# JeffOwOSun/ntm-tracker

Measured on AMD Instinct MI355X. Metric: frames/sec (whole node) VGG16+NTM(128x20) seq_len=20, higher is better.
Workload: dtype f32

## Files before the change

### include/ntmtrack.h

```cpp
#ifndef NTMTRACK_H_
#define NTMTRACK_H_

#include <stddef.h>
#include <stdint.h>

#ifdef __cplusplus
extern "C" {
#endif

#define NTK_OK               0
#define NTK_ERR_BAD_SHAPE   -1
#define NTK_ERR_BAD_PTR     -2
#define NTK_ERR_UNSUPPORTED -3
#define NTK_ERR_HIP         -4

int ntk_version(void);
const char* ntk_last_error(void);


int ntk_vgg_packed_k(int cin);
int ntk_vgg_pack_weights(const float* w_hwio, float* w_packed, int cin, int cout, void* stream);

int ntk_vgg_conv3x3_relu_f32(const float* in, const float* w_packed, const float* bias,
                             float* out, int frames, int H, int W, int cin, int cout,
// ... 29 lines not shown
int ntk_vgg_pack_weights_wino43(const float* w_hwio, float* u_packed, int cin, int cout, void* stream);
int ntk_vgg_conv3x3_relu_wino43_f32(const float* in, const float* u_packed, const float* bias, float* out,
                                    int frames, int H, int W, int cin, int cout, int fuse_pool, void* stream);
int ntk_vgg_conv3x3_relu_wino43_window_f32(const float* in, const float* u_packed, const float* bias, float* out,
                                           int frames, int H, int W, int cin, int cout, int fuse_pool,
                                           int y0, int x0, int y1, int x1, void* stream);
int ntk_vgg_conv3x3_relu_wino43_form_f32(const float* in, const float* u_packed, const float* bias, float* out,
                                         int frames, int H, int W, int cin, int cout, int fuse_pool,
                                         int y0, int x0, int y1, int x1, int waves, void* stream);
int ntk_vgg_conv3x3_relu_wino43_layout_f32(const float* in, const float* u_packed, const float* bias, float* out,
                                           int frames, int H, int W, int cin, int cout, int fuse_pool,
                                           int in_blocked, int out_blocked, void* stream);

int ntk_maxpool2x2(const float* in, float* out, int frames, int H, int W, int C, void* stream);


int ntk_gemm_nt_f32(const float* A, int lda, const float* B, int ldb, const float* bias,
                    float* C, int ldc, int M, int N, int K, void* stream);

size_t ntk_gemm_tn_workspace_bytes(int M, int N, int splits);
int ntk_gemm_tn_f32(const float* A, int lda, const float* B, int ldb, float* C, int ldc,
                    int M, int N, int K, int splits, int accumulate, float* workspace,
                    void* stream);

int ntk_transpose_pad(const float* in, int ldi, float* out, int ldo, int rows, int cols, void* stream);


int ntk_ntm_padded_dims(int N, int Md, int R, int Wh, int hid, int shift_range, int O,
                        int* P, int* PP, int* K, int* ldz, int* ldh);

#define NTK_NTM_FWD_WS           1
#define NTK_NTM_FWD_FIX512       2
#define NTK_NTM_FWD_GENERIC768   3
#define NTK_NTM_FWD_GENERIC1024  4
#define NTK_NTM_FWD_FIX640_DEV   5
#define NTK_NTM_BWD_WS           1
#define NTK_NTM_BWD_FIX          2
#define NTK_NTM_BWD_GENERIC768   3
#define NTK_NTM_BWD_GENERIC1024  4
#define NTK_NTM_PLAN_FWD 1
#define NTK_NTM_PLAN_BWD 2

int ntk_ntm_seq_plan(int B, int N, int Md, int R, int Wh, int hid, int shift_range, int O, int write_first,
                     int ldkT, int ldhT, int* fwd_kernel, int* fwd_threads, int* bwd_kernel, int* bwd_threads);

int ntk_ntm_seq_fwd(int B, int S, int N, int Md, int R, int Wh, int hid, int shift_range, int O,
// ... 128 lines not shown
                             float* st_wc, float* st_wv, float* st_w, float* st_M, float* st_read,
                             float* st_xtop, float* st_buf0, float* st_bufk, float* st_lgates, float* st_lc,
                             void* stream);
int ntk_ntm_seq_bwd_deep_sim(int B, int S, int N, int Md, int R, int Wh, int hid, int shift_range, int O, int L,
                             int write_first, int similarity,
                             const float* Wb, const float* WaT, int ldhT,
                             const float* M0, const float* w0, const float* cs0,
                             const float* st_gates, const float* st_c, const float* st_u,
                             const float* st_wc, const float* st_wv, const float* st_w, const float* st_M,
                             const float* st_lgates, const float* st_lc,
                             const float* dlogits,
                             const float* dM_fin, const float* dw_fin, const float* dread_fin, const float* dcs_fin,
                             float* dgates, float* dpre, float* du, float* dM0, float* dw0, float* dread0, float* dcs0,
                             void* stream);

int ntk_lstm_step_fwd(const float* pre, const float* c_prev, float forget_bias, float* c, float* h, float* act,
                      int B, int hid, void* stream);
int ntk_lstm_step_bwd(const float* act, const float* c_prev, const float* c, const float* dh, const float* dc,
                      float* dpre, float* dc_prev, int B, int hid, void* stream);

int ntk_ntm_init_state(const float* v, float* out, int n, int B, int act, void* stream);
int ntk_ntm_init_state_bwd(const float* v, const float* dout, float* dv, int n, int B, int act,
                           int accumulate, void* stream);

int ntk_dnc_padded_dims(int N, int W, int R, int Wn, int hid, int O,
                        int* I, int* IP, int* K, int* ldz, int* ldh, int* Ky, int* ldy, int* OP);
int ntk_dnc_seq_fwd(int B, int S, int N, int W, int R, int Wn, int hid, int O, float clip_value,
                    const float* xproj, const float* Wr, const float* Wi, const float* Wy,
                    float* mem, float* link, float* usage, float* rw, float* ww, float* prec,
                    float* reads, float* hc, float* out,
                    float* rec_z, float* rec_gates, float* rec_c, float* rec_hc, float* rec_yin,
                    float* rec_ifc, float* rec_u, float* rec_ww, float* rec_rw, float* rec_cw,
                    float* rec_cr, float* rec_al, float* rec_p, float* rec_fwd, float* rec_bwd,
                    float* rec_M, float* rec_L, float* rec_ypre, void* stream);

int ntk_dnc_cluster_plan(int B, int N, int W, int R, int Wn, int hid, int O, int k_request, int* k, size_t* workspace_bytes);
int ntk_dnc_cluster_status(const void* workspace, int B, int k, void* stream);
int ntk_dnc_cluster_placement(const void* workspace, int B, int k, int* same_xcd_clusters, void* stream);
int ntk_dnc_cluster_guard(const void* workspace, size_t workspace_bytes, int mp_form, int B, int k, float* loss, float* grad,
                          size_t n, void* stream);
int ntk_dnc_cluster_inject_abort(void* workspace, size_t workspace_bytes, int mp_form, int B, int k, void* stream);
int ntk_dnc_cluster_fwd(int B, int S, int N, int W, int R, int Wn, int hid, int O, float clip_value, int k,
                        const float* xproj, const float* Wr, const float* Wi, const float* Wy,
                        float* mem, float* link, float* usage, float* rw, float* ww, float* prec,
                        float* reads, float* hc, float* out,
                        float* rec_z, float* rec_gates, float* rec_c, float* rec_hc, float* rec_yin,
// ... 166 lines not shown
```

### ntm-tracker_amd/_lib.py

```python
import ctypes
import os

import torch

_HERE = os.path.dirname(os.path.abspath(__file__))
LIB_PATH = os.environ.get("NTK_LIB_PATH") or os.path.join(_HERE, "libntmtrack_hip.so")

_lib = None


class NtkError(RuntimeError):
    pass


def _sig(lib):
    c_int, c_void_p, c_size_t = ctypes.c_int, ctypes.c_void_p, ctypes.c_size_t
    P = c_void_p
    sigs = {
        "ntk_version": (c_int, []),
        "ntk_last_error": (ctypes.c_char_p, []),
        "ntk_vgg_packed_k": (c_int, [c_int]),
        "ntk_vgg_pack_weights": (c_int, [P, P, c_int, c_int, P]),
        "ntk_vgg_conv3x3_relu_f32": (c_int, [P, P, P, P, c_int, c_int, c_int, c_int, c_int, c_int, P]),
        "ntk_vgg_pack_weights_bf16": (c_int, [P, P, c_int, c_int, P]),
        "ntk_vgg_conv3x3_relu_bf16": (c_int, [P, P, P, P] + [c_int] * 7 + [P]),
        "ntk_vgg_conv3x3_relu_f32_to_bf16": (c_int, [P, P, P, P] + [c_int] * 5 + [P]),
        "ntk_vgg_bf16p_packed_elems": (c_size_t, [c_int, c_int]),
        "ntk_vgg_bf16p_supported": (c_int, [c_int] * 5),
        "ntk_vgg_pack_weights_bf16p": (c_int, [P, P] + [c_int] * 4 + [P]),
        "ntk_vgg_conv3x3_relu_bf16p": (c_int, [P, P, P, P] + [c_int] * 7 + [P]),
        "ntk_vgg_split3_packed_elems": (c_size_t, [c_int, c_int]),
        "ntk_vgg_split3_supported": (c_int, [c_int] * 5),
        "ntk_vgg_pack_weights_split3": (c_int, [P, P] + [c_int] * 4 + [P]),
        "ntk_vgg_conv3x3_relu_split3": (c_int, [P, P, P, P] + [c_int] * 8 + [P]),
        "ntk_gemm_nt_f32": (c_int, [P, c_int, P, c_int, P, P, c_int, c_int, c_int, c_int, P]),
        "ntk_gemm_tn_workspace_bytes": (c_size_t, [c_int, c_int, c_int]),
        "ntk_gemm_tn_f32": (c_int, [P, c_int, P, c_int, P, c_int, c_int, c_int, c_int, c_int, c_int, P, P]),
        "ntk_ntm_padded_dims": (c_int, [c_int] * 7 + [ctypes.POINTER(c_int)] * 5),
        "ntk_ntm_seq_fwd": (c_int, [c_int] * 10 + [P] * 23 + [P]),
        "ntk_transpose_pad": (c_int, [P, c_int, P, c_int, c_int, c_int, P]),
        "ntk_ntm_seq_bwd": (c_int, [c_int] * 10 + [P, c_int, P, c_int] + [P] * 21 + [P]),
        "ntk_ntm_seq_deep_supported": (c_int, [c_int] * 9),
        "ntk_ntm_seq_plan": (c_int, [c_int] * 11 + [ctypes.POINTER(c_int)] * 4),
        "ntk_ntm_seq_deep_plan": (c_int, [c_int] * 10 + [ctypes.POINTER(c_int)] * 4),
        "ntk_ntm_seq_deep_packed_floats": (c_int, [c_int] * 5 + [ctypes.POINTER(c_size_t)] * 3),
        "ntk_ntm_seq_deep_pack": (c_int, [c_int] * 5 + [P] * 6 + [P]),
        "ntk_ntm_seq_fwd_deep": (c_int, [c_int] * 12 + [P] * 29 + [P]),
        "ntk_ntm_seq_bwd_deep": (c_int, [c_int] * 11 + [P, P, c_int] + [P] * 24 + [P]),
        "ntk_dnc_padded_dims": (c_int, [c_int] * 6 + [ctypes.POINTER(c_int)] * 8),
        "ntk_dnc_seq_fwd": (c_int, [c_int] * 8 + [ctypes.c_float] + [P] * 13 + [P] * 18 + [P]),
        "ntk_dnc_cluster_plan": (c_int, [c_int] * 8 + [ctypes.POINTER(c_int), ctypes.POINTER(c_size_t)]),
        "ntk_dnc_cluster_status": (c_int, [P, c_int, c_int, P]),
        "ntk_dnc_cluster_placement": (c_int, [P, c_int, c_int, P, P]),
        "ntk_dnc_cluster_guard": (c_int, [P, c_size_t, c_int, c_int, c_int, P, P, c_size_t, P]),
        "ntk_dnc_cluster_inject_abort": (c_int, [P, c_size_t, c_int, c_int, c_int, P]),
        "ntk_dnc_cluster_fwd": (c_int, [c_int] * 8 + [ctypes.c_float, c_int] + [P] * 13 + [P] * 18 + [P, P]),
        "ntk_dnc_cluster_bwd_plan": (c_int, [c_int] * 8 + [ctypes.POINTER(c_int), ctypes.POINTER(c_size_t)]),
        "ntk_dnc_cluster_bwd": (c_int, [c_int] * 8 + [ctypes.c_float, c_int] + [P, c_int, P, P] + [P] * 7 + [P] * 15 + [P] * 6 + [P, c_int, P, P]),
        "ntk_cu_count": (c_int, []),
        "ntk_dnc_mp_plan": (c_int, [c_int] * 8 + [ctypes.POINTER(c_int), ctypes.POINTER(c_size_t)]),
# ... 45 lines not shown
        "ntk_vgg_conv3x3_relu_wino43_form_f32": (c_int, [P] * 4 + [c_int] * 11 + [P]),
        "ntk_vgg_conv3x3_relu_wino43_layout_f32": (c_int, [P] * 4 + [c_int] * 8 + [P]),
        "ntk_maxpool2x2": (c_int, [P, P] + [c_int] * 4 + [P]),
        "ntk_offset_loss_fwd": (c_int, [P] * 4 + [c_int] * 4 + [P]),
        "ntk_offset_loss_bwd": (c_int, [P] * 3 + [c_int] * 4 + [P]),
        "ntk_dnc_seq_bwd": (c_int, [c_int] * 8 + [ctypes.c_float] + [P, c_int, P, c_int, P] + [P] * 7 + [P] * 15 + [P] * 6 + [P, c_int, P]),
        "ntk_gather_serialize": (c_int, [P, P, P] + [c_int] * 9 + [P]),
        "ntk_gather_serialize_online": (c_int, [P, P, P] + [c_int] * 9 + [P]),
        "ntk_crop_and_resize": (c_int, [P, c_int, c_int, c_int, P] + [ctypes.c_float] * 4 + [P, c_int, c_int, ctypes.c_float, P]),
        "ntk_crop_and_resize_batch": (c_int, [P] + [c_int] * 5 + [P, P, P, P] + [c_int] * 3 + [ctypes.c_float, P]),
        "ntk_track_boxes_update": (c_int, [P, c_int, c_int, ctypes.c_double, ctypes.c_double] + [P] * 6 + [P]),
        "ntk_track_overlap_scores": (c_int, [P, P, P, P, c_int, c_int, c_int, P, c_int, P, c_int, P, P, P]),
        "ntk_select_rows": (c_int, [P, P, P, P, c_int, c_int, P]),
        "ntk_dnc_state_keep": (c_int, [P, c_int, c_int, c_int, P, P, P, P]),
        "ntk_resize_bilinear": (c_int, [P, c_int, c_int, c_int, P, c_int, c_int, P]),
        "ntk_offset_loss": (c_int, [P, P, P, P, P, c_int, c_int, c_int, c_int, P]),
        "ntk_log_loss": (c_int, [P, P, P, P, c_int, P]),
        "ntk_serialize_sequential": (c_int, [P, P, P] + [c_int] * 5 + [P]),
        "ntk_heatmap_ce_loss": (c_int, [P] * 5 + [c_int] * 3 + [P]),
        "ntk_serialize_two_step": (c_int, [P, P, P] + [c_int] * 5 + [P]),
        "ntk_two_step_ce_loss": (c_int, [P] * 5 + [c_int] * 3 + [P]),
        "ntk_ntm_init_state": (c_int, [P, P, c_int, c_int, c_int, P]),
        "ntk_ntm_init_state_bwd": (c_int, [P, P, P, c_int, c_int, c_int, c_int, P]),
        "ntk_global_norm_workspace_bytes": (c_size_t, [c_size_t]),
        "ntk_global_norm": (c_int, [P, c_size_t, P, P, P]),
        "ntk_rmsprop_clip_step": (c_int, [P, P, P, P, c_size_t] + [ctypes.c_float] * 5 + [P, P]),
        "ntk_rmsprop_clip_step_checked": (c_int, [P, P, P, P, c_size_t] + [ctypes.c_float] * 5 + [P, P, P, P]),
    }
    for name, (res, args) in sigs.items():
        fn = getattr(lib, name)
        fn.restype = res
        fn.argtypes = args
    return sigs


def lib():
    global _lib
    if _lib is None:
        if not os.path.exists(LIB_PATH):
            raise NtkError(
                "libntmtrack_hip.so is not built (%s). Run `python -c 'import __graft_entry__ as g; g.build()'` "
                "or `make -C ntm-tracker_amd/csrc`. There is no CPU fallback." % LIB_PATH)
        l = ctypes.CDLL(LIB_PATH)
        l._ntk_sigs = _sig(l)
        _lib = l
    return _lib
# ... 25 lines not shown
```

### ntm-tracker_amd/csrc/head_opt.hip

```cpp
#include "common.h"

namespace {

__global__ void gather_serialize_kernel(const float* __restrict__ fmap, const float* __restrict__ gts0,
                                        float* __restrict__ X, int T, int Hf, int Wf, int C, int ldx,
                                        int g0, int gstep, int gn, int delim_first) {
    const int NF = gn * gn;
    const int row = blockIdx.x;
    const int pos = row % (NF + 1);
    const int i = delim_first ? (pos == 0 ? NF : pos - 1) : pos;
    const int ft = row / (NF + 1);
    const int t = ft % T, b = ft / T;
    float* xr = X + (size_t)row * ldx;
    const int C4 = C >> 2;
    if (i < NF) {
        const int y = g0 + (i / gn) * gstep, x = g0 + (i % gn) * gstep;
        const f32x4* src = reinterpret_cast<const f32x4*>(fmap + (((size_t)ft * Hf + y) * Wf + x) * C);
        f32x4* dst = reinterpret_cast<f32x4*>(xr);
        for (int c = threadIdx.x; c < C4; c += blockDim.x) dst[c] = src[c];
    } else {
        f32x4 z = {0.f, 0.f, 0.f, 0.f};
        f32x4* dst = reinterpret_cast<f32x4*>(xr);
        for (int c = threadIdx.x; c < C4; c += blockDim.x) dst[c] = z;
    }
// ... 180 lines not shown
}

__global__ __launch_bounds__(1024) void log_loss_kernel(const float* __restrict__ logits, const float* __restrict__ labels,
                                                         float* __restrict__ loss, float* __restrict__ dlogits, int n) {
    __shared__ float red[16];
    const float eps = 1e-7f, inv = 1.0f / (float)n;
    float acc = 0.f;
    for (int i = threadIdx.x; i < n; i += blockDim.x) {
        const float p = 1.0f / (1.0f + expf(-logits[i]));
        const float y = labels[i];
        acc += -(y * logf(p + eps) + (1.0f - y) * logf(1.0f - p + eps));
        if (dlogits) dlogits[i] = inv * (-(y / (p + eps)) + (1.0f - y) / (1.0f - p + eps)) * p * (1.0f - p);
    }
    acc = wave_sum(acc);
    if ((threadIdx.x & 63) == 0) red[threadIdx.x >> 6] = acc;
    __syncthreads();
    if (threadIdx.x == 0) {
        float s = 0.f;
        for (int w = 0; w < (int)(blockDim.x >> 6); ++w) s += red[w];
        *loss = s * inv;
    }
}

__global__ void init_state_kernel(const float* __restrict__ v, float* __restrict__ out, int n, int B, int act) {
    const int i = blockIdx.x * blockDim.x + threadIdx.x;
    if (i >= n) return;
    const float x = v[i];
    const float y = act ? 1.0f / (1.0f + expf(-x)) : tanhf(x);
    for (int b = 0; b < B; ++b) out[(size_t)b * n + i] = y;
}

__global__ void init_state_bwd_kernel(const float* __restrict__ v, const float* __restrict__ dout,
                                      float* __restrict__ dv, int n, int B, int act, int accumulate) {
    const int i = blockIdx.x * blockDim.x + threadIdx.x;
    if (i >= n) return;
    float s = 0.f;
    for (int b = 0; b < B; ++b) s += dout[(size_t)b * n + i];
    const float x = v[i];
    float dy;
    if (act) { const float y = 1.0f / (1.0f + expf(-x)); dy = y * (1.0f - y); }
    else { const float y = tanhf(x); dy = 1.0f - y * y; }
    const float g = s * dy;
    dv[i] = accumulate ? dv[i] + g : g;
}

constexpr int SUMSQ_BLOCK = 256;
constexpr int SUMSQ_PER_BLOCK = 4096;

__global__ void sumsq_partial_kernel(const float* __restrict__ g, float* __restrict__ partial, size_t n) {
    __shared__ float red[SUMSQ_BLOCK / 64];
    const size_t base = (size_t)blockIdx.x * SUMSQ_PER_BLOCK;
    float acc = 0.f;
    for (int i = threadIdx.x; i < SUMSQ_PER_BLOCK; i += SUMSQ_BLOCK) {
        const size_t idx = base + i;
        if (idx < n) { const float v = g[idx]; acc += v * v; }
    }
    acc = wave_sum(acc);
    if ((threadIdx.x & 63) == 0) red[threadIdx.x >> 6] = acc;
    __syncthreads();
    if (threadIdx.x == 0) {
        float s = 0.f;
        for (int w = 0; w < SUMSQ_BLOCK / 64; ++w) s += red[w];
        partial[blockIdx.x] = s;
    }
}

// ... 442 lines not shown
    const unsigned nb = (unsigned)((total + 255) / 256 < 4096 ? (total + 255) / 256 : 4096);
    serialize_two_step_kernel<<<nb, 256, 0, (hipStream_t)stream>>>(feat, target, X, B, T, D, F, ldx);
    NTK_CHECK_LAUNCH("ntk_serialize_two_step");
    return NTK_OK;
}

extern "C" int ntk_two_step_ce_loss(const float* logits, const float* gt, float* probs, float* loss, float* dlogits,
                                    int B, int T, int F, void* stream) {
    NTK_REQUIRE(logits && gt && (loss || dlogits || probs), NTK_ERR_BAD_PTR, "ntk_two_step_ce_loss: null pointer");
    NTK_REQUIRE(B > 0 && T >= 1 && F > 0, NTK_ERR_BAD_SHAPE, "ntk_two_step_ce_loss: B=%d T=%d F=%d", B, T, F);
    two_step_ce_loss_kernel<<<1, 1024, 0, (hipStream_t)stream>>>(logits, gt, probs, loss, dlogits, B, T, F);
    NTK_CHECK_LAUNCH("ntk_two_step_ce_loss");
    return NTK_OK;
}

extern "C" int ntk_ntm_init_state(const float* v, float* out, int n, int B, int act, void* stream) {
    NTK_REQUIRE(v && out, NTK_ERR_BAD_PTR, "ntk_ntm_init_state: null pointer");
    NTK_REQUIRE(n > 0 && B > 0 && (act == 0 || act == 1), NTK_ERR_BAD_SHAPE, "ntk_ntm_init_state: n=%d B=%d act=%d", n, B, act);
    init_state_kernel<<<(n + 255) / 256, 256, 0, (hipStream_t)stream>>>(v, out, n, B, act);
    NTK_CHECK_LAUNCH("ntk_ntm_init_state");
    return NTK_OK;
}

extern "C" int ntk_ntm_init_state_bwd(const float* v, const float* dout, float* dv, int n, int B, int act,
                                      int accumulate, void* stream) {
    NTK_REQUIRE(v && dout && dv, NTK_ERR_BAD_PTR, "ntk_ntm_init_state_bwd: null pointer");
    NTK_REQUIRE(n > 0 && B > 0 && (act == 0 || act == 1), NTK_ERR_BAD_SHAPE, "ntk_ntm_init_state_bwd: n=%d B=%d act=%d", n, B, act);
    init_state_bwd_kernel<<<(n + 255) / 256, 256, 0, (hipStream_t)stream>>>(v, dout, dv, n, B, act, accumulate);
    NTK_CHECK_LAUNCH("ntk_ntm_init_state_bwd");
    return NTK_OK;
}

extern "C" size_t ntk_global_norm_workspace_bytes(size_t n) {
    return ((n + SUMSQ_PER_BLOCK - 1) / SUMSQ_PER_BLOCK) * sizeof(float);
}

extern "C" int ntk_global_norm(const float* grads, size_t n, float* workspace, float* gnorm, void* stream) {
    NTK_REQUIRE(grads && workspace && gnorm, NTK_ERR_BAD_PTR, "ntk_global_norm: null pointer");
    NTK_REQUIRE(n > 0, NTK_ERR_BAD_SHAPE, "ntk_global_norm: n=0");
    const int nb = (int)((n + SUMSQ_PER_BLOCK - 1) / SUMSQ_PER_BLOCK);
    sumsq_partial_kernel<<<nb, SUMSQ_BLOCK, 0, (hipStream_t)stream>>>(grads, workspace, n);
    NTK_CHECK_LAUNCH("ntk_global_norm(partial)");
    sumsq_final_kernel<<<1, 1024, 0, (hipStream_t)stream>>>(workspace, nb, gnorm);
    NTK_CHECK_LAUNCH("ntk_global_norm(final)");
    return NTK_OK;
}
// ... 25 lines not shown
```

### ntm-tracker_amd/dnc.py

```python
import collections
import ctypes

import torch

from . import _lib
from .ntm import gemm_nt, gemm_tn

_P = _lib.ptr

DNCState = collections.namedtuple("DNCState", ("access_output", "access_state", "controller_state"))
AccessState = collections.namedtuple("AccessState", ("memory", "read_weights", "write_weights", "linkage", "usage"))
TemporalLinkageState = collections.namedtuple("TemporalLinkageState", ("link", "precedence_weights"))
LSTMState = collections.namedtuple("LSTMState", ("hidden", "cell"))

INTERFACE = ("write_vectors", "erase_vectors", "free_gate", "allocation_gate", "write_gate", "read_mode",
             "write_keys", "write_strengths", "read_keys", "read_strengths")


class FlatParams(object):

    def __init__(self, shapes, device):
        n = 0
        self.shapes = list(shapes)
        self.offsets = {}
        for name, shp in shapes:
            sz = 1
            for s_ in shp:
                sz *= s_
            n = (n + 3) // 4 * 4
# ... 431 lines not shown
            return _P(keep[-1])
        recs = (_P(rec["gates"]), _P(rec["c"]), _P(rec["ifc"]), _P(rec["u"]), _P(rec["ww"]), _P(rec["rw"]), _P(rec["cw"]),
                _P(rec["cr"]), _P(rec["al"]), _P(rec["p"]), _P(rec["fwd"]), _P(rec["bwd"]), _P(rec["M"]), _P(rec["L"]),
                _P(rec["ypre"]), _P(dout), _P(gM), _P(gL), _P(dgates), _P(dxi), _P(dypre),
                _P(gcarry) if gcarry is not None else None, 1 if carry_in else 0)
        state0 = (c(acc.memory), c(acc.linkage.link), c(acc.usage), c(acc.read_weights), c(acc.write_weights),
                  c(acc.linkage.precedence_weights), _P(hc0))
        plan = self._cluster_bwd_plan(B)
        self.last_cluster_bwd_k = plan[1] if plan else 1
        self.last_cluster_bwd_form = plan[0] if plan else None
        if plan:
            fn = _lib.lib().ntk_dnc_cluster_bwd if plan[0] == "lds" else _lib.lib().ntk_dnc_mp_bwd
            _lib.check(fn(B, S, self.N, self.W, self.R, self.Wn, hid, self.O, self.clip_value, plan[1],
                          _P(WrT), ldkT, _P(self.Wi), _P(self.Wy), *state0, *recs, _P(plan[2]), _lib.stream()),
                       "ntk_dnc_cluster_bwd" if plan[0] == "lds" else "ntk_dnc_mp_bwd")
        else:
            _lib.check(_lib.lib().ntk_dnc_seq_bwd(
                B, S, self.N, self.W, self.R, self.Wn, hid, self.O, self.clip_value,
                _P(WrT), ldkT, _P(WiT), ldhT, _P(self.Wy), *state0, *recs, _lib.stream()), "ntk_dnc_seq_bwd")
        return dgates, dxi, dypre

    def _weight_grads(self, X2, rec, dgates, dxi, dypre, BS, accumulate):
        P, hid = self.params, self.hid
        gemm_tn(dgates.view(BS, 4 * hid), X2, P.view("WxT", grad=True), accumulate=accumulate)
        gemm_tn(rec["z"].view(BS, self.ldz), dgates.view(BS, 4 * hid), P.view("Wr", grad=True), accumulate=accumulate)
        gemm_tn(rec["hc"].view(BS, self.ldh), dxi.view(BS, self.IP), P.view("Wi", grad=True), accumulate=accumulate)
        gemm_tn(rec["yin"].view(BS, self.ldy), dypre.view(BS, self.OP), P.view("Wy", grad=True), accumulate=accumulate)

    def backward_sequence(self, X, dout, unpack=True):
        if not 1 <= self.Wn <= 4:
            raise _lib.NtkError("DNC BPTT on the HIP path implements 1..4 write heads (got %d)" % self.Wn)
        rec, st0 = self.last_record, self.last_initial
        if not rec and not self.last_segments:
            raise _lib.NtkError("backward_sequence needs a recorded forward pass (record=True)")
        B, S, _ = X.shape
        dev, L, stream = self.device, _lib.lib(), _lib.stream()
        hid = self.hid
        ldkT, ldhT = (self.K + 3) // 4 * 4, (hid + 3) // 4 * 4
        WrT = torch.empty((4 * hid, ldkT), device=dev)
        WiT = torch.empty((self.IP, ldhT), device=dev)
        _lib.check(L.ntk_transpose_pad(_P(self.Wr), 4 * hid, _P(WrT), ldkT, self.K, 4 * hid, stream), "ntk_transpose_pad")
        _lib.check(L.ntk_transpose_pad(_P(self.Wi), self.IP, _P(WiT), ldhT, hid, self.IP, stream), "ntk_transpose_pad")
        gM = torch.zeros((B, self.N, self.W), device=dev)
        gL = torch.zeros((B, self.Wn, self.N, self.N), device=dev)
        dout = dout.contiguous()
        if not self.last_segments:
            dgates, dxi, dypre = self._launch_bwd(B, S, st0, rec, dout, WrT, ldkT, WiT, ldhT, gM, gL, None, False)
            self._weight_grads(X.view(B * S, self.ldx), rec, dgates, dxi, dypre, B * S, False)
            return self._unpack(grad=True) if unpack else None
        xp, ckpt, bounds, fwd_recs, seg_cap = self.last_segments
# ... 424 lines not shown
```

### ntm-tracker_amd/ntm.py

```python
import ctypes
import os

import torch

from . import _lib

_P = _lib.ptr


def _np(t):
    return None if t is None else _lib.ptr(t)


class NTMDims(object):
    def __init__(self, input_dim, output_dim, mem_size, mem_dim, shift_range, hidden, read_heads, write_heads):
        self.D = int(input_dim)
        self.O = int(output_dim)
        self.N, self.Md = int(mem_size), int(mem_dim)
        self.R, self.Wh = int(read_heads), int(write_heads)
        self.H = self.R + self.Wh
        self.hid = int(hidden)
        self.shift_range = int(shift_range)
        self.SS = 2 * self.shift_range + 1
        vals = [ctypes.c_int() for _ in range(5)]
# ... 90 lines not shown
            "init_state/read": self.view("V_r", grad).cpu().clone(),
        }


def gemm_nt(A, B, bias=None, out=None):
    M, K = A.shape
    N, K2 = B.shape
    assert K == K2
    if out is None:
        out = torch.empty((M, N), device=A.device, dtype=torch.float32)
    _lib.check(_lib.lib().ntk_gemm_nt_f32(_P(A), A.stride(0), _P(B), B.stride(0), _np(bias), _P(out), out.stride(0),
                                          M, N, K, _lib.stream()), "ntk_gemm_nt_f32")
    return out


_WS = {}


def gemm_tn(A, B, out, accumulate=False, splits=None, workspace=None):
    K, M = A.shape
    K2, N = B.shape
    assert K == K2 and tuple(out.shape) == (M, N)
    if splits is None:
        tiles = ((M + 127) // 128) * ((N + 127) // 128)
        splits = max(1, min((K + 255) // 256, (1024 + tiles - 1) // tiles))
    L = _lib.lib()
    need = L.ntk_gemm_tn_workspace_bytes(M, N, splits) // 4
    if workspace is None or workspace.numel() < need:
        workspace = _WS.get(A.device)
        if workspace is None or workspace.numel() < need:
            workspace = torch.empty(need, device=A.device, dtype=torch.float32)
            _WS[A.device] = workspace
    _lib.check(L.ntk_gemm_tn_f32(_P(A), A.stride(0), _P(B), B.stride(0), _P(out), out.stride(0), M, N, K, splits,
                                 1 if accumulate else 0, _P(workspace), _lib.stream()), "ntk_gemm_tn_f32")
    return out


SIMILARITY_MODES = {"as_coded": 0, "smooth_cosine": 1}


def similarity_mode(similarity):
    if similarity not in SIMILARITY_MODES:
        raise _lib.NtkError("similarity=%r: expected one of %s" % (similarity, ", ".join(sorted(SIMILARITY_MODES))))
    return SIMILARITY_MODES[similarity]


class NTMCell(object):

    def __new__(cls, output_dim=None, mem_size=128, mem_dim=20, shift_range=1, controller_hidden_size=100,
                controller_num_layers=10, *args, **kwargs):
        if cls is NTMCell and controller_num_layers != 1:
            return object.__new__(StackedNTMCell)
        return object.__new__(cls)

    def __init__(self, output_dim, mem_size=128, mem_dim=20, shift_range=1,
                 controller_hidden_size=100, controller_num_layers=10,
                 write_head_size=3, read_head_size=3, write_first=False,
                 input_dim=None, device="cuda", init_scale=0.1, seed=None, similarity="as_coded"):
# ... 34 lines not shown
                "lstm/cell_0/weights": u(d.D + d.RM + d.hid, 4 * d.hid),
                "lstm/cell_0/biases": torch.zeros(4 * d.hid),
                "addressing/weights": u(d.hid, d.P), "addressing/biases": torch.zeros(d.P),
                "output/weights": u(d.hid, d.O), "output/biases": torch.zeros(d.O),
                "init_state/M": u(d.N, d.Md), "init_state/w": u(d.H, d.N), "init_state/read": u(d.R, d.Md),
            }
        self.params.load_tf(tf_state_dict)

    def load_state_dict(self, sd, input_dim=None):
        if input_dim is None:
            input_dim = sd["lstm/cell_0/weights"].shape[0] - self.read_head_size * self.mem_dim - self.controller_hidden_size
        self._build(int(input_dim), sd)

    def state_dict(self, grad=False):
        return self.params.to_tf(grad)

    input_ldx = property(lambda self: self.dims.ldx)

    def zero_state(self, batch_size, initializer=None):
        d, dev, L = self.dims, self.device, _lib.lib()
        if d is None:
            raise _lib.NtkError("zero_state before the cell has parameters: pass input_dim= or load_state_dict()")
        st = self.state_placeholder(batch_size)
        for name, key, act in (("V_M", "M", 0), ("V_w", "w", 1), ("V_r", "read", 0)):
            v = self.params.view(name)
            _lib.check(L.ntk_ntm_init_state(_P(v), _P(st[key]), v.numel(), batch_size, act, _lib.stream()),
                       "ntk_ntm_init_state")
        st["controller_state"].zero_()
        return st

    def state_placeholder(self, batch_size):
        d, dev = self.dims, self.device
        return {
            "M": torch.empty((batch_size, d.N, d.Md), device=dev),
            "w": torch.empty((batch_size, d.H, d.N), device=dev),
            "read": torch.empty((batch_size, d.R, d.Md), device=dev),
            "controller_state": torch.empty((batch_size, 2 * d.hid), device=dev),
        }

    FWD_KERNELS = {0: None, 1: "ws", 2: "fixdims-512", 3: "generic-768", 4: "generic-1024", 5: "fixdims-640-dev"}
    BWD_KERNELS = {0: None, 1: "ws", 2: "fix", 3: "generic-768", 4: "generic-1024"}

    def plan(self, batch):
        d = self.dims
        if d is None:
            raise _lib.NtkError("plan before the cell has parameters: pass input_dim= or load_state_dict()")
# ... 68 lines not shown
        WaT = torch.empty((d.PP, ldhT), device=dev)
        st = _lib.stream()
        _lib.check(L.ntk_transpose_pad(_P(P.view("Wr")), 4 * d.hid, _P(WrT), ldkT, d.K, 4 * d.hid, st), "ntk_transpose_pad")
        _lib.check(L.ntk_transpose_pad(_P(P.view("Wa")), d.PP, _P(WaT), ldhT, d.hid, d.PP, st), "ntk_transpose_pad")
        dgates = torch.empty((B, S, 4 * d.hid), device=dev)
        du = torch.empty((B, S, d.PP), device=dev)
        g0 = self.state_placeholder(B)
        df = dfinal or {}
        keep = []

        def cp(t):
            keep.append(t.contiguous())
            return _P(keep[-1])
        _lib.check(L.ntk_ntm_seq_bwd_sim(
            B, S, d.N, d.Md, d.R, d.Wh, d.hid, d.shift_range, d.O, 1 if self.write_first else 0, self._sim,
            _P(WrT), ldkT, _P(WaT), ldhT,
            cp(state0["M"]), cp(state0["w"]), cp(state0["controller_state"]),
            _P(rec["gates"]), _P(rec["c"]), _P(rec["u"]), _P(rec["wc"]), _P(rec["wv"]), _P(rec["w"]), _P(rec["M"]),
            cp(dlogits),
            _np(df.get("M")), _np(df.get("w")), _np(df.get("read")), _np(df.get("controller_state")),
            _P(dgates), _P(du), _P(g0["M"]), _P(g0["w"]), _P(g0["read"]), _P(g0["controller_state"]), st),
            "ntk_ntm_seq_bwd")
        BS = B * S
        gemm_tn(dgates.view(BS, 4 * d.hid), X.view(BS, d.ldx), P.view("WxT", grad=True), workspace=workspace)
        gemm_tn(rec["z"].view(BS, d.ldz), dgates.view(BS, 4 * d.hid), P.view("Wr", grad=True), workspace=workspace)
        gemm_tn(rec["h"].view(BS, d.ldh), du.view(BS, d.PP), P.view("Wa", grad=True), workspace=workspace)
        self.last_dX = None
        if self.want_input_grad:
            Wx = torch.empty((d.ldx, 4 * d.hid), device=dev)
            _lib.check(L.ntk_transpose_pad(_P(P.view("WxT")), d.ldx, _P(Wx), 4 * d.hid, 4 * d.hid, d.ldx, st), "ntk_transpose_pad")
            self.last_dX = gemm_nt(dgates.view(BS, 4 * d.hid), Wx).view(B, S, d.ldx)
        return g0

    def init_state_backward(self, g0, batch_size):
        L = _lib.lib()
        for name, key, act in (("V_M", "M", 0), ("V_w", "w", 1), ("V_r", "read", 0)):
            v = self.params.view(name)
            _lib.check(L.ntk_ntm_init_state_bwd(_P(v), _P(g0[key]), _P(self.params.view(name, grad=True)),
                                                v.numel(), batch_size, act, 0, _lib.stream()), "ntk_ntm_init_state_bwd")

    def __call__(self, inputs, prev_state, M_prev=None, w_prev=None, read_prev=None,
                 controller_state=None, scope=None):
        if self.dims is None:
            self._build(inputs.shape[1])
        d = self.dims
        if prev_state is not None:
            M_prev, w_prev = prev_state["M"], prev_state["w"]
            read_prev, controller_state = prev_state["read"], prev_state["controller_state"]
        st = {"M": M_prev, "w": w_prev, "read": read_prev, "controller_state": controller_state}
        X = self._pad_inputs(inputs.unsqueeze(1))
        logits, outputs, new, rec = self.run_sequence(X, st, record=True)
        u = rec["u"][:, 0]
        B = inputs.shape[0]
        H, Md, R = d.H, d.Md, d.R
        w = rec["w"][:, 0]
        k = u[:, d.oK:d.oB].reshape(B, H, Md)
        from . import ops as _ops
        Mp, wp = M_prev.contiguous().float(), w_prev.contiguous().float()
# ... 515 lines not shown
```

Baseline: 13920.

## Group weight-gradient GEMMs and init-state kernels into single launches

Adds a grouped split-K TN GEMM kernel that runs several weight-gradient problems in one launch, followed by a single grouped slab reduction. The NTM and DNC backward passes use it instead of issuing one gemm_tn per weight. The three or four per-tensor init_state forward and backward launches are also merged into one kernel each. The aim is to cut launch count and tail idle time in small backward GEMMs. The cost is a new GEMM kernel with different tiling (160x128) whose efficiency may differ from the existing one, plus an environment switch to fall back.

```diff
diff --git a/include/ntmtrack.h b/include/ntmtrack.h
--- a/include/ntmtrack.h
+++ b/include/ntmtrack.h
@@ -75,6 +75,19 @@
 int ntk_gemm_tn_f32(const float* A, int lda, const float* B, int ldb, float* C, int ldc,
                     int M, int N, int K, int splits, int accumulate, float* workspace,
                     void* stream);
+
+#define NTK_GEMM_TN_GROUP_MAX 8
+typedef struct ntk_gemm_tn_problem {
+    const float* A;
+    const float* B;
+    float* C;
+    int lda, ldb, ldc;
+    int M, N, K;
+    int splits, accumulate;
+    size_t slab_offset;
+} ntk_gemm_tn_problem;
+int ntk_gemm_tn_grouped_f32(const ntk_gemm_tn_problem* problems, int count, float* workspace,
+                            size_t workspace_floats, void* stream);
 
 int ntk_transpose_pad(const float* in, int ldi, float* out, int ldo, int rows, int cols, void* stream);
 
@@ -249,6 +262,11 @@
 int ntk_ntm_init_state(const float* v, float* out, int n, int B, int act, void* stream);
 int ntk_ntm_init_state_bwd(const float* v, const float* dout, float* dv, int n, int B, int act,
                            int accumulate, void* stream);
+int ntk_ntm_init_state3(const float* vM, const float* vw, const float* vr, float* M, float* w, float* read,
+                        float* controller_state, int nM, int nw, int nr, int nc, int B, void* stream);
+int ntk_ntm_init_state_bwd3(const float* vM, const float* vw, const float* vr, const float* gM, const float* gw,
+                            const float* gr, float* dM, float* dw, float* dr, int nM, int nw, int nr, int B,
+                            int accumulate, void* stream);
 
 int ntk_dnc_padded_dims(int N, int W, int R, int Wn, int hid, int O,
                         int* I, int* IP, int* K, int* ldz, int* ldh, int* Ky, int* ldy, int* OP);
diff --git a/ntm-tracker_amd/_lib.py b/ntm-tracker_amd/_lib.py
--- a/ntm-tracker_amd/_lib.py
+++ b/ntm-tracker_amd/_lib.py
@@ -11,6 +11,18 @@
 
 class NtkError(RuntimeError):
     pass
+
+
+class GemmTnProblem(ctypes.Structure):
+    _fields_ = [("A", ctypes.c_void_p), ("B", ctypes.c_void_p), ("C", ctypes.c_void_p),
+                ("lda", ctypes.c_int), ("ldb", ctypes.c_int), ("ldc", ctypes.c_int),
+                ("M", ctypes.c_int), ("N", ctypes.c_int), ("K", ctypes.c_int),
+                ("splits", ctypes.c_int), ("accumulate", ctypes.c_int), ("slab_offset", ctypes.c_size_t)]
+
+
+GEMM_TN_GROUP_MAX = 8
+
+CORE_TAIL_SEPARATE = os.environ.get("NTK_CORE_TAIL", "") == "separate"
 
 
 def _sig(lib):
@@ -36,6 +48,7 @@
         "ntk_gemm_nt_f32": (c_int, [P, c_int, P, c_int, P, P, c_int, c_int, c_int, c_int, P]),
         "ntk_gemm_tn_workspace_bytes": (c_size_t, [c_int, c_int, c_int]),
         "ntk_gemm_tn_f32": (c_int, [P, c_int, P, c_int, P, c_int, c_int, c_int, c_int, c_int, c_int, P, P]),
+        "ntk_gemm_tn_grouped_f32": (c_int, [ctypes.POINTER(GemmTnProblem), c_int, P, c_size_t, P]),
         "ntk_ntm_padded_dims": (c_int, [c_int] * 7 + [ctypes.POINTER(c_int)] * 5),
         "ntk_ntm_seq_fwd": (c_int, [c_int] * 10 + [P] * 23 + [P]),
         "ntk_transpose_pad": (c_int, [P, c_int, P, c_int, c_int, c_int, P]),
@@ -127,6 +140,8 @@
         "ntk_two_step_ce_loss": (c_int, [P] * 5 + [c_int] * 3 + [P]),
         "ntk_ntm_init_state": (c_int, [P, P, c_int, c_int, c_int, P]),
         "ntk_ntm_init_state_bwd": (c_int, [P, P, P, c_int, c_int, c_int, c_int, P]),
+        "ntk_ntm_init_state3": (c_int, [P] * 7 + [c_int] * 5 + [P]),
+        "ntk_ntm_init_state_bwd3": (c_int, [P] * 9 + [c_int] * 5 + [P]),
         "ntk_global_norm_workspace_bytes": (c_size_t, [c_size_t]),
         "ntk_global_norm": (c_int, [P, c_size_t, P, P, P]),
         "ntk_rmsprop_clip_step": (c_int, [P, P, P, P, c_size_t] + [ctypes.c_float] * 5 + [P, P]),
diff --git a/ntm-tracker_amd/csrc/gemm_grouped.hip b/ntm-tracker_amd/csrc/gemm_grouped.hip
--- /dev/null
+++ b/ntm-tracker_amd/csrc/gemm_grouped.hip
@@ -0,0 +1,205 @@
+#include "common.h"
+
+namespace {
+
+constexpr int GK = 32;
+constexpr int GM = 160, GN = 128;
+constexpr int GU = GM / 32;
+constexpr int GTILE = GK * (GM + GN);
+constexpr int GA4 = GM / 4;
+
+struct TnProb {
+    const float* A;
+    const float* B;
+    float* slab;
+    float* C;
+    int lda, ldb, ldc, M, N, K, kchunk, splits, accumulate;
+    int mtiles, ntiles;
+    int block_end;
+    int elem_end;
+};
+
+struct TnGroup {
+    TnProb p[NTK_GEMM_TN_GROUP_MAX];
+    int count;
+};
+
+__device__ __attribute__((aligned(16))) float g_tn_zero[4];
+
+__device__ __forceinline__ void tn_dma16(const float* src, float* lds_wave_base) {
+    __builtin_amdgcn_global_load_lds((const __attribute__((address_space(1))) void*)src,
+                                     (__attribute__((address_space(3))) void*)lds_wave_base, 16, 0, 0);
+}
+
+template <int NU>
+__device__ __forceinline__ void tn_tile(const TnProb& P, int m0, int n0, int z, float* lds) {
+    const int tid = threadIdx.x, lane = tid & 63, wave = tid >> 6;
+    const int kbeg = z * P.kchunk;
+    const int kend = min(P.K, kbeg + P.kchunk);
+    const int nk = kend > kbeg ? (kend - kbeg + GK - 1) / GK : 0;
+    const bool active = n0 + wave * 32 < P.N;
+    float* As = lds;
+    float* Bs = lds + GK * GM;
+
+    const float* pa[GU];
+    const float* pb[4];
+    int ka[GU], kb[4];
+#pragma unroll
+    for (int s = 0; s < GU; ++s) {
+        const int e = tid + 256 * s, kr = e / GA4, c = m0 + (e - kr * GA4) * 4;
+        ka[s] = c < P.M ? kr : 2 * GK + P.kchunk;
+        pa[s] = P.A + (size_t)(kbeg + kr) * P.lda + c;
+    }
+#pragma unroll
+    for (int s = 0; s < 4; ++s) {
+        const int kr = (tid >> 5) + 8 * s, c = n0 + (tid & 31) * 4;
+        kb[s] = c < P.N ? kr : 2 * GK + P.kchunk;
+        pb[s] = P.B + (size_t)(kbeg + kr) * P.ldb + c;
+    }
+    auto issue = [&](int kt) {
+        const int left = kend - kbeg - kt * GK;
+#pragma unroll
+        for (int s = 0; s < GU; ++s)
+            tn_dma16(ka[s] < left ? pa[s] + (size_t)kt * GK * P.lda : g_tn_zero, As + (256 * s + 64 * wave) * 4);
+#pragma unroll
+        for (int s = 0; s < 4; ++s)
+            tn_dma16(kb[s] < left ? pb[s] + (size_t)kt * GK * P.ldb : g_tn_zero, Bs + (256 * s + 64 * wave) * 4);
+    };
+
+    f32x16 acc[NU];
+#pragma unroll
+    for (int u = 0; u < NU; ++u)
+#pragma unroll
+        for (int r = 0; r < 16; ++r) acc[u][r] = 0.f;
+
+    const int i = lane & 31, kh = lane >> 5;
+    const float* ap = As + kh * GM + i;
+    const float* bp = Bs + kh * GN + wave * 32 + i;
+    for (int kt = 0; kt < nk; ++kt) {
+        if (kt > 0) __syncthreads();
+        issue(kt);
+        asm volatile("s_waitcnt vmcnt(0)" ::: "memory");
+        __syncthreads();
+        if (active) {
+#pragma unroll
+            for (int s = 0; s < GK / 2; ++s) {
+                float a[NU];
+                const float b = bp[2 * s * GN];
+#pragma unroll
+                for (int u = 0; u < NU; ++u) a[u] = ap[2 * s * GM + u * 32];
+#pragma unroll
+                for (int u = 0; u < NU; ++u) acc[u] = __builtin_amdgcn_mfma_f32_32x32x2f32(a[u], b, acc[u], 0, 0, 0);
+            }
+        }
+    }
+    if (!active) return;
+    const int n = n0 + wave * 32 + i;
+    if (n >= P.N) return;
+    float* out = P.slab + (size_t)z * P.M * P.N;
+#pragma unroll
+    for (int u = 0; u < NU; ++u)
+#pragma unroll
+        for (int r = 0; r < 16; ++r) {
+            const int m = m0 + u * 32 + 4 * kh + (r & 3) + 8 * (r >> 2);
+            if (m < P.M) out[(size_t)m * P.N + n] = acc[u][r];
+        }
+}
+
+__global__ __launch_bounds__(256, 4) void gemm_tn_grouped_kernel(const TnGroup G) {
+    __shared__ __attribute__((aligned(1024))) float lds[GTILE];
+    int pi = 0;
+    while (pi + 1 < G.count && (int)blockIdx.x >= G.p[pi].block_end) ++pi;
+    const TnProb& P = G.p[pi];
+    const int b = blockIdx.x - (pi ? G.p[pi - 1].block_end : 0);
+    const int tiles = P.mtiles * P.ntiles;
+    const int li = b >> 3;
+    const int z = (li / tiles) * 8 + (b & 7), t = li % tiles;
+    if (z >= P.splits) return;
+    const int nt = t / P.mtiles, mt = t - nt * P.mtiles;
+    const int m0 = mt * GM, n0 = nt * GN;
+    const int nu = min(GU, (P.M - m0 + 31) / 32);
+    switch (nu) {
+        case 1: tn_tile<1>(P, m0, n0, z, lds); break;
+        case 2: tn_tile<2>(P, m0, n0, z, lds); break;
+        case 3: tn_tile<3>(P, m0, n0, z, lds); break;
+        case 4: tn_tile<4>(P, m0, n0, z, lds); break;
+        default: tn_tile<5>(P, m0, n0, z, lds); break;
+    }
+}
+
+__global__ void slab_reduce_grouped_kernel(const TnGroup G) {
+    const int idx = blockIdx.x * blockDim.x + threadIdx.x;
+    if (idx >= G.p[G.count - 1].elem_end) return;
+    int pi = 0;
+    while (pi + 1 < G.count && idx >= G.p[pi].elem_end) ++pi;
+    const TnProb& P = G.p[pi];
+    const int e = idx - (pi ? G.p[pi - 1].elem_end : 0);
+    const int m = e / P.N, n = e - m * P.N;
+    const size_t mn = (size_t)P.M * P.N;
+    const float* sp = P.slab + e;
+    float s = 0.f;
+    int z = 0;
+    for (; z + 8 <= P.splits; z += 8) {
+        float v[8];
+#pragma unroll
+        for (int j = 0; j < 8; ++j) v[j] = sp[(size_t)(z + j) * mn];
+#pragma unroll
+        for (int j = 0; j < 8; ++j) s += v[j];
+    }
+    for (; z < P.splits; ++z) s += sp[(size_t)z * mn];
+    float* c = P.C + (size_t)m * P.ldc + n;
+    *c = P.accumulate ? (*c + s) : s;
+}
+
+}
+
+extern "C" int ntk_gemm_tn_grouped_f32(const ntk_gemm_tn_problem* problems, int count, float* workspace,
+                                       size_t workspace_floats, void* stream) {
+    NTK_REQUIRE(problems && workspace, NTK_ERR_BAD_PTR, "ntk_gemm_tn_grouped_f32: null pointer");
+    NTK_REQUIRE(count > 0 && count <= NTK_GEMM_TN_GROUP_MAX, NTK_ERR_BAD_SHAPE,
+                "ntk_gemm_tn_grouped_f32: %d problems (1 .. %d per launch)", count, NTK_GEMM_TN_GROUP_MAX);
+    TnGroup G;
+    G.count = count;
+    long blocks = 0, elems = 0;
+    for (int i = 0; i < count; ++i) {
+        const ntk_gemm_tn_problem& q = problems[i];
+        NTK_REQUIRE(q.A && q.B && q.C, NTK_ERR_BAD_PTR, "ntk_gemm_tn_grouped_f32: problem %d: null pointer", i);
+        NTK_REQUIRE(ntk_aligned16(q.A) && ntk_aligned16(q.B), NTK_ERR_BAD_PTR,
+                    "ntk_gemm_tn_grouped_f32: problem %d: A, B must be 16-byte aligned", i);
+        NTK_REQUIRE(q.M > 0 && q.N > 0 && q.K > 0 && q.splits > 0 && q.splits <= 65535 && (q.M % 4) == 0 && (q.N % 4) == 0 &&
+                        (q.lda % 4) == 0 && (q.ldb % 4) == 0 && q.lda >= q.M && q.ldb >= q.N && q.ldc >= q.N,
+                    NTK_ERR_BAD_SHAPE,
+                    "ntk_gemm_tn_grouped_f32: problem %d: M=%d N=%d K=%d splits=%d lda=%d ldb=%d ldc=%d (M, N, lda, ldb multiples of 4)",
+                    i, q.M, q.N, q.K, q.splits, q.lda, q.ldb, q.ldc);
+        const size_t need = (size_t)q.M * q.N * q.splits;
+        NTK_REQUIRE(q.slab_offset <= workspace_floats && need <= workspace_floats - q.slab_offset, NTK_ERR_BAD_SHAPE,
+                    "ntk_gemm_tn_grouped_f32: problem %d: slabs [%zu, %zu) exceed the workspace of %zu floats", i,
+                    q.slab_offset, q.slab_offset + need, workspace_floats);
+        for (int j = 0; j < i; ++j) {
+            const size_t o = problems[j].slab_offset, n = (size_t)problems[j].M * problems[j].N * problems[j].splits;
+            NTK_REQUIRE(q.slab_offset >= o + n || o >= q.slab_offset + need, NTK_ERR_BAD_SHAPE,
+                        "ntk_gemm_tn_grouped_f32: slabs of problems %d and %d overlap", j, i);
+        }
+        TnProb& P = G.p[i];
+        P.A = q.A; P.B = q.B; P.C = q.C; P.slab = workspace + q.slab_offset;
+        P.lda = q.lda; P.ldb = q.ldb; P.ldc = q.ldc; P.M = q.M; P.N = q.N; P.K = q.K;
+        P.splits = q.splits; P.accumulate = q.accumulate ? 1 : 0;
+        int kchunk = (q.K + q.splits - 1) / q.splits;
+        P.kchunk = ((kchunk + GK - 1) / GK) * GK;
+        P.mtiles = (q.M + GM - 1) / GM;
+        P.ntiles = (q.N + GN - 1) / GN;
+        blocks += (long)P.mtiles * P.ntiles * ((q.splits + 7) / 8 * 8);
+        elems += (long)q.M * q.N;
+        NTK_REQUIRE(blocks < 2147483647L && elems < 2147483647L - 256, NTK_ERR_BAD_SHAPE,
+                    "ntk_gemm_tn_grouped_f32: %ld workgroups / %ld elements exceed the grid's index range", blocks, elems);
+        P.block_end = (int)blocks;
+        P.elem_end = (int)elems;
+    }
+    for (int i = count; i < NTK_GEMM_TN_GROUP_MAX; ++i) G.p[i] = G.p[count - 1];
+    hipStream_t st = (hipStream_t)stream;
+    gemm_tn_grouped_kernel<<<(unsigned)blocks, 256, 0, st>>>(G);
+    NTK_CHECK_LAUNCH("ntk_gemm_tn_grouped_f32");
+    slab_reduce_grouped_kernel<<<(unsigned)((elems + 255) / 256), 256, 0, st>>>(G);
+    NTK_CHECK_LAUNCH("ntk_gemm_tn_grouped_f32(reduce)");
+    return NTK_OK;
+}
diff --git a/ntm-tracker_amd/csrc/head_opt.hip b/ntm-tracker_amd/csrc/head_opt.hip
--- a/ntm-tracker_amd/csrc/head_opt.hip
+++ b/ntm-tracker_amd/csrc/head_opt.hip
@@ -226,18 +226,14 @@
     }
 }
 
-__global__ void init_state_kernel(const float* __restrict__ v, float* __restrict__ out, int n, int B, int act) {
-    const int i = blockIdx.x * blockDim.x + threadIdx.x;
-    if (i >= n) return;
+__device__ __forceinline__ void init_state_elem(const float* __restrict__ v, float* __restrict__ out, int i, int n, int B, int act) {
     const float x = v[i];
     const float y = act ? 1.0f / (1.0f + expf(-x)) : tanhf(x);
     for (int b = 0; b < B; ++b) out[(size_t)b * n + i] = y;
 }
 
-__global__ void init_state_bwd_kernel(const float* __restrict__ v, const float* __restrict__ dout,
-                                      float* __restrict__ dv, int n, int B, int act, int accumulate) {
-    const int i = blockIdx.x * blockDim.x + threadIdx.x;
-    if (i >= n) return;
+__device__ __forceinline__ void init_state_bwd_elem(const float* __restrict__ v, const float* __restrict__ dout,
+                                                    float* __restrict__ dv, int i, int n, int B, int act, int accumulate) {
     float s = 0.f;
     for (int b = 0; b < B; ++b) s += dout[(size_t)b * n + i];
     const float x = v[i];
@@ -246,6 +242,44 @@
     else { const float y = tanhf(x); dy = 1.0f - y * y; }
     const float g = s * dy;
     dv[i] = accumulate ? dv[i] + g : g;
+}
+
+__global__ void init_state_kernel(const float* __restrict__ v, float* __restrict__ out, int n, int B, int act) {
+    const int i = blockIdx.x * blockDim.x + threadIdx.x;
+    if (i < n) init_state_elem(v, out, i, n, B, act);
+}
+
+__global__ void init_state_bwd_kernel(const float* __restrict__ v, const float* __restrict__ dout,
+                                      float* __restrict__ dv, int n, int B, int act, int accumulate) {
+    const int i = blockIdx.x * blockDim.x + threadIdx.x;
+    if (i < n) init_state_bwd_elem(v, dout, dv, i, n, B, act, accumulate);
+}
+
+struct InitState3 {
+    const float* v[3];
+    float* out[3];
+    const float* dout[3];
+    int n[3];
+};
+
+__global__ void init_state3_kernel(const InitState3 a, float* __restrict__ ctrl, int nc, int B) {
+    int i = blockIdx.x * blockDim.x + threadIdx.x;
+    if (i < a.n[0]) { init_state_elem(a.v[0], a.out[0], i, a.n[0], B, 0); return; }
+    i -= a.n[0];
+    if (i < a.n[1]) { init_state_elem(a.v[1], a.out[1], i, a.n[1], B, 1); return; }
+    i -= a.n[1];
+    if (i < a.n[2]) { init_state_elem(a.v[2], a.out[2], i, a.n[2], B, 0); return; }
+    i -= a.n[2];
+    if (i < nc) for (int b = 0; b < B; ++b) ctrl[(size_t)b * nc + i] = 0.f;
+}
+
+__global__ void init_state_bwd3_kernel(const InitState3 a, int B, int accumulate) {
+    int i = blockIdx.x * blockDim.x + threadIdx.x;
+    if (i < a.n[0]) { init_state_bwd_elem(a.v[0], a.dout[0], a.out[0], i, a.n[0], B, 0, accumulate); return; }
+    i -= a.n[0];
+    if (i < a.n[1]) { init_state_bwd_elem(a.v[1], a.dout[1], a.out[1], i, a.n[1], B, 1, accumulate); return; }
+    i -= a.n[1];
+    if (i < a.n[2]) init_state_bwd_elem(a.v[2], a.dout[2], a.out[2], i, a.n[2], B, 0, accumulate);
 }
 
 constexpr int SUMSQ_BLOCK = 256;
@@ -734,6 +768,31 @@
     return NTK_OK;
 }
 
+extern "C" int ntk_ntm_init_state3(const float* vM, const float* vw, const float* vr, float* M, float* w, float* read,
+                                   float* controller_state, int nM, int nw, int nr, int nc, int B, void* stream) {
+    NTK_REQUIRE(vM && vw && vr && M && w && read && controller_state, NTK_ERR_BAD_PTR, "ntk_ntm_init_state3: null pointer");
+    NTK_REQUIRE(nM > 0 && nw > 0 && nr > 0 && nc > 0 && B > 0 && (long)nM + nw + nr + nc < 2147483647L - 256, NTK_ERR_BAD_SHAPE,
+                "ntk_ntm_init_state3: nM=%d nw=%d nr=%d nc=%d B=%d", nM, nw, nr, nc, B);
+    InitState3 a = {{vM, vw, vr}, {M, w, read}, {nullptr, nullptr, nullptr}, {nM, nw, nr}};
+    const int total = nM + nw + nr + nc;
+    init_state3_kernel<<<(total + 255) / 256, 256, 0, (hipStream_t)stream>>>(a, controller_state, nc, B);
+    NTK_CHECK_LAUNCH("ntk_ntm_init_state3");
+    return NTK_OK;
+}
+
+extern "C" int ntk_ntm_init_state_bwd3(const float* vM, const float* vw, const float* vr, const float* gM, const float* gw,
+                                       const float* gr, float* dM, float* dw, float* dr, int nM, int nw, int nr, int B,
+                                       int accumulate, void* stream) {
+    NTK_REQUIRE(vM && vw && vr && gM && gw && gr && dM && dw && dr, NTK_ERR_BAD_PTR, "ntk_ntm_init_state_bwd3: null pointer");
+    NTK_REQUIRE(nM > 0 && nw > 0 && nr > 0 && B > 0 && (long)nM + nw + nr < 2147483647L - 256, NTK_ERR_BAD_SHAPE,
+                "ntk_ntm_init_state_bwd3: nM=%d nw=%d nr=%d B=%d", nM, nw, nr, B);
+    InitState3 a = {{vM, vw, vr}, {dM, dw, dr}, {gM, gw, gr}, {nM, nw, nr}};
+    const int total = nM + nw + nr;
+    init_state_bwd3_kernel<<<(total + 255) / 256, 256, 0, (hipStream_t)stream>>>(a, B, accumulate);
+    NTK_CHECK_LAUNCH("ntk_ntm_init_state_bwd3");
+    return NTK_OK;
+}
+
 extern "C" int ntk_ntm_init_state_bwd(const float* v, const float* dout, float* dv, int n, int B, int act,
                                       int accumulate, void* stream) {
     NTK_REQUIRE(v && dout && dv, NTK_ERR_BAD_PTR, "ntk_ntm_init_state_bwd: null pointer");
diff --git a/ntm-tracker_amd/dnc.py b/ntm-tracker_amd/dnc.py
--- a/ntm-tracker_amd/dnc.py
+++ b/ntm-tracker_amd/dnc.py
@@ -4,7 +4,7 @@
 import torch
 
 from . import _lib
-from .ntm import gemm_nt, gemm_tn
+from .ntm import gemm_nt, gemm_tn, gemm_tn_grouped
 
 _P = _lib.ptr
 
@@ -482,10 +482,15 @@
 
     def _weight_grads(self, X2, rec, dgates, dxi, dypre, BS, accumulate):
         P, hid = self.params, self.hid
-        gemm_tn(dgates.view(BS, 4 * hid), X2, P.view("WxT", grad=True), accumulate=accumulate)
-        gemm_tn(rec["z"].view(BS, self.ldz), dgates.view(BS, 4 * hid), P.view("Wr", grad=True), accumulate=accumulate)
-        gemm_tn(rec["hc"].view(BS, self.ldh), dxi.view(BS, self.IP), P.view("Wi", grad=True), accumulate=accumulate)
-        gemm_tn(rec["yin"].view(BS, self.ldy), dypre.view(BS, self.OP), P.view("Wy", grad=True), accumulate=accumulate)
+        wgrads = ((dgates.view(BS, 4 * hid), X2, P.view("WxT", grad=True), accumulate),
+                  (rec["z"].view(BS, self.ldz), dgates.view(BS, 4 * hid), P.view("Wr", grad=True), accumulate),
+                  (rec["hc"].view(BS, self.ldh), dxi.view(BS, self.IP), P.view("Wi", grad=True), accumulate),
+                  (rec["yin"].view(BS, self.ldy), dypre.view(BS, self.OP), P.view("Wy", grad=True), accumulate))
+        if _lib.CORE_TAIL_SEPARATE:
+            for A_, B_, out_, acc_ in wgrads:
+                gemm_tn(A_, B_, out_, accumulate=acc_)
+        else:
+            gemm_tn_grouped(wgrads)
 
     def backward_sequence(self, X, dout, unpack=True):
         if not 1 <= self.Wn <= 4:
diff --git a/ntm-tracker_amd/ntm.py b/ntm-tracker_amd/ntm.py
--- a/ntm-tracker_amd/ntm.py
+++ b/ntm-tracker_amd/ntm.py
@@ -136,8 +136,7 @@
     K2, N = B.shape
     assert K == K2 and tuple(out.shape) == (M, N)
     if splits is None:
-        tiles = ((M + 127) // 128) * ((N + 127) // 128)
-        splits = max(1, min((K + 255) // 256, (1024 + tiles - 1) // tiles))
+        splits = _default_splits(M, N, K)
     L = _lib.lib()
     need = L.ntk_gemm_tn_workspace_bytes(M, N, splits) // 4
     if workspace is None or workspace.numel() < need:
@@ -148,6 +147,46 @@
     _lib.check(L.ntk_gemm_tn_f32(_P(A), A.stride(0), _P(B), B.stride(0), _P(out), out.stride(0), M, N, K, splits,
                                  1 if accumulate else 0, _P(workspace), _lib.stream()), "ntk_gemm_tn_f32")
     return out
+
+
+def _default_splits(M, N, K):
+    tiles = ((M + 127) // 128) * ((N + 127) // 128)
+    return max(1, min((K + 255) // 256, (1024 + tiles - 1) // tiles))
+
+
+def gemm_tn_grouped(problems, workspace=None):
+    L = _lib.lib()
+    if not 0 < len(problems) <= _lib.GEMM_TN_GROUP_MAX:
+        raise _lib.NtkError("gemm_tn_grouped: %d problems (1 .. %d per launch)" % (len(problems), _lib.GEMM_TN_GROUP_MAX))
+    table = (_lib.GemmTnProblem * len(problems))()
+    rows, off = [], 0
+    for prob in problems:
+        A, B, out = prob[:3]
+        accumulate = bool(prob[3]) if len(prob) > 3 else False
+        splits = prob[4] if len(prob) > 4 and prob[4] is not None else None
+        K, M = A.shape
+        K2, N = B.shape
+        assert K == K2 and tuple(out.shape) == (M, N)
+        for t in (A, B, out):
+            if not t.is_cuda or t.dtype != torch.float32 or t.stride(1) != 1:
+                raise _lib.NtkError("gemm_tn_grouped: expected fp32 device tensors with contiguous rows")
+        if splits is None:
+            splits = _default_splits(M, N, K)
+        rows.append((A, B, out, M, N, K, splits, accumulate, off))
+        off += M * N * splits
+    rows.sort(key=lambda r: -((r[3] + 31) // 32) * ((r[4] + 31) // 32) * r[5])
+    for q, (A, B, out, M, N, K, splits, accumulate, o) in zip(table, rows):
+        q.A, q.B, q.C = A.data_ptr(), B.data_ptr(), out.data_ptr()
+        q.lda, q.ldb, q.ldc = A.stride(0), B.stride(0), out.stride(0)
+        q.M, q.N, q.K, q.splits, q.accumulate, q.slab_offset = M, N, K, splits, 1 if accumulate else 0, o
+    dev = problems[0][0].device
+    if workspace is None or workspace.numel() < off:
+        workspace = _WS.get(dev)
+        if workspace is None or workspace.numel() < off:
+            workspace = torch.empty(off, device=dev, dtype=torch.float32)
+            _WS[dev] = workspace
+    _lib.check(L.ntk_gemm_tn_grouped_f32(table, len(problems), _P(workspace), workspace.numel(), _lib.stream()),
+               "ntk_gemm_tn_grouped_f32")
 
 
 SIMILARITY_MODES = {"as_coded": 0, "smooth_cosine": 1}
@@ -228,6 +267,12 @@
         if d is None:
             raise _lib.NtkError("zero_state before the cell has parameters: pass input_dim= or load_state_dict()")
         st = self.state_placeholder(batch_size)
+        if not _lib.CORE_TAIL_SEPARATE:
+            vM, vw, vr = (self.params.view(n) for n in ("V_M", "V_w", "V_r"))
+            _lib.check(L.ntk_ntm_init_state3(_P(vM), _P(vw), _P(vr), _P(st["M"]), _P(st["w"]), _P(st["read"]),
+                                             _P(st["controller_state"]), vM.numel(), vw.numel(), vr.numel(), 2 * d.hid,
+                                             batch_size, _lib.stream()), "ntk_ntm_init_state3")
+            return st
         for name, key, act in (("V_M", "M", 0), ("V_w", "w", 1), ("V_r", "read", 0)):
             v = self.params.view(name)
             _lib.check(L.ntk_ntm_init_state(_P(v), _P(st[key]), v.numel(), batch_size, act, _lib.stream()),
@@ -342,9 +387,14 @@
             _P(dgates), _P(du), _P(g0["M"]), _P(g0["w"]), _P(g0["read"]), _P(g0["controller_state"]), st),
             "ntk_ntm_seq_bwd")
         BS = B * S
-        gemm_tn(dgates.view(BS, 4 * d.hid), X.view(BS, d.ldx), P.view("WxT", grad=True), workspace=workspace)
-        gemm_tn(rec["z"].view(BS, d.ldz), dgates.view(BS, 4 * d.hid), P.view("Wr", grad=True), workspace=workspace)
-        gemm_tn(rec["h"].view(BS, d.ldh), du.view(BS, d.PP), P.view("Wa", grad=True), workspace=workspace)
+        wgrads = ((dgates.view(BS, 4 * d.hid), X.view(BS, d.ldx), P.view("WxT", grad=True)),
+                  (rec["z"].view(BS, d.ldz), dgates.view(BS, 4 * d.hid), P.view("Wr", grad=True)),
+                  (rec["h"].view(BS, d.ldh), du.view(BS, d.PP), P.view("Wa", grad=True)))
+        if _lib.CORE_TAIL_SEPARATE:
+            for A_, B_, out_ in wgrads:
+                gemm_tn(A_, B_, out_, workspace=workspace)
+        else:
+            gemm_tn_grouped(wgrads, workspace=workspace)
         self.last_dX = None
         if self.want_input_grad:
             Wx = torch.empty((d.ldx, 4 * d.hid), device=dev)
@@ -354,6 +404,14 @@
 
     def init_state_backward(self, g0, batch_size):
         L = _lib.lib()
+        if not _lib.CORE_TAIL_SEPARATE:
+            P = self.params
+            vM, vw, vr = (P.view(n) for n in ("V_M", "V_w", "V_r"))
+            _lib.check(L.ntk_ntm_init_state_bwd3(_P(vM), _P(vw), _P(vr), _P(g0["M"]), _P(g0["w"]), _P(g0["read"]),
+                                                 _P(P.view("V_M", grad=True)), _P(P.view("V_w", grad=True)),
+                                                 _P(P.view("V_r", grad=True)), vM.numel(), vw.numel(), vr.numel(),
+                                                 batch_size, 0, _lib.stream()), "ntk_ntm_init_state_bwd3")
+            return
         for name, key, act in (("V_M", "M", 0), ("V_w", "w", 1), ("V_r", "read", 0)):
             v = self.params.view(name)
             _lib.check(L.ntk_ntm_init_state_bwd(_P(v), _P(g0[key]), _P(self.params.view(name, grad=True)),
```

Measured after the change: 13950, median of 6. No clear change (+0.2%).
